# meijieru/AtomNAS

Hardware: AMD Instinct MI355X
Metric: images/sec (whole node) AtomNAS-C supernet 224x224 bs256/GPU (higher is better)
Workload: dtype bf16; 1 GPU; atomnas_c_supernet full training step (fwd + CE-smooth/L2/L1 + bwd + grad all-reduce + RMSprop + EMA), 224x224; per_gpu_batch=256, global_batch=256, parallelism=dp1, hip_graph=True

## Files before the change

### atomnas_amd/csrc/pwconv_tn.hip

```cpp
#include "pwconv.h"

namespace atomnas {

constexpr int UT_MAX = 20;
constexpr int TN_ROWS = 32;

template <typename T, int UMODE, int VMODE>
__global__ __launch_bounds__(256) void k_gemm_tn(Operand U, int NU, Operand V, int NV, float* __restrict__ out, long si, long sj,
                                                 long M, long rows_per_block, float* __restrict__ ws) {
  using MM = Mma<T>;
  constexpr int E = MM::EPL;
  constexpr int SUB = TN_ROWS / (4 * E);
  constexpr int UP = 16 * UT_MAX + 2;
  constexpr int VP = 64 + 2;
  __shared__ T s_u[TN_ROWS * UP];
  __shared__ T s_v[TN_ROWS * VP];

  const int tid = threadIdx.x;
  const int lane = tid & 63, wave = tid >> 6;
  const int q = lane >> 4, j = lane & 15;

  const int u0 = blockIdx.z * (16 * UT_MAX);
  const int nu = min(NU - u0, 16 * UT_MAX);
  const int ut = (nu + 15) / 16;
  const int v0 = blockIdx.y * 64;
  const int nv = min(NV - v0, 64);
  const long r_beg = (long)blockIdx.x * rows_per_block;
  const long r_end = min(M, r_beg + rows_per_block);

  f32x4 acc[UT_MAX];
#pragma unroll
  for (int t = 0; t < UT_MAX; ++t) acc[t] = f32x4{0.f, 0.f, 0.f, 0.f};

  const int ugroups = (ut * 16) / E;
  const int vgroups = 64 / E;

  for (long r0 = r_beg; r0 < r_end; r0 += TN_ROWS) {
    for (int idx = tid; idx < TN_ROWS * ugroups; idx += 256) {
      const int rr = idx / ugroups, cg = (idx % ugroups) * E;
      float v[E];
      load_pro<T, UMODE>(U, r0 + rr, (r0 + rr) < r_end, u0 + cg, NU, v);
#pragma unroll
      for (int e = 0; e < E; ++e) s_u[rr * UP + cg + e] = from_f32<T>(v[e]);
    }
    for (int idx = tid; idx < TN_ROWS * vgroups; idx += 256) {
      const int rr = idx / vgroups, cg = (idx % vgroups) * E;
      float v[E];
      load_pro<T, VMODE>(V, r0 + rr, (r0 + rr) < r_end, v0 + cg, NV, v);
#pragma unroll
      for (int e = 0; e < E; ++e) s_v[rr * VP + cg + e] = from_f32<T>(v[e]);
    }
    __syncthreads();

#pragma unroll
    for (int sb = 0; sb < SUB; ++sb) {
      float bv[E];
#pragma unroll
      for (int e = 0; e < E; ++e) bv[e] = to_f32(s_v[(4 * E * sb + E * q + e) * VP + 16 * wave + j]);
      const typename MM::frag bf = MM::pack(bv);
#pragma unroll
      for (int t = 0; t < UT_MAX; ++t) {
        if (t < ut) {
          float uv[E];
#pragma unroll
          for (int e = 0; e < E; ++e) uv[e] = to_f32(s_u[(4 * E * sb + E * q + e) * UP + 16 * t + j]);
          acc[t] = MM::mma(MM::pack(uv), bf, acc[t]);
        }
      }
    }
    __syncthreads();
  }

  const int vc = v0 + 16 * wave + j;
  if (vc < NV) {
#pragma unroll
    for (int t = 0; t < UT_MAX; ++t) {
      if (t < ut) {
#pragma unroll
        for (int r = 0; r < 4; ++r) {
          const int uc = u0 + 16 * t + 4 * q + r;
          if (uc < NU) {
            if (ws) ws[((long)blockIdx.x * NU + uc) * NV + vc] = acc[t][r];
            else out[uc * si + vc * sj] += acc[t][r];
          }
        }
      }
    }
  }
}


template <int UMODE, int VMODE, int UTT, int VTT, int ROWS>
__global__ __launch_bounds__(256) void k_gemm_tn2(Operand U, int NU, Operand V, int NV, float* __restrict__ out, long si, long sj, long M,
                                                  long rows_per_block, int nchunks, int vt, int uz, int xcd_aware, float* __restrict__ ws) {
  using T = bf16_t;
  using MM = Mma<T>;
  constexpr int VW = 64 * VTT;
  constexpr int RP = ROWS + 8;
  extern __shared__ __attribute__((aligned(16))) unsigned char smem_raw[];
  T* s_v = reinterpret_cast<T*>(smem_raw);
  T* s_u = s_v + VW * RP;
  float* s_cv = reinterpret_cast<float*>(s_u + 16 * UTT * RP);
  float* s_cu = s_cv + 3 * VW;

  const int tid = threadIdx.x;
  const int lane = tid & 63, wave = tid >> 6;
  const int q = lane >> 4, j = lane & 15;
  const int ntile = vt * uz;
  int tile; long chunk;
  if (xcd_aware) {
    const int b_xcd = blockIdx.x & 7, b_local = blockIdx.x >> 3;
    tile = b_local % ntile;
    chunk = (long)(b_local / ntile) * 8 + b_xcd;
  } else {
    chunk = blockIdx.x % nchunks;
    tile = blockIdx.x / nchunks;
    if (tile >= ntile) return;
  }
  if (chunk >= nchunks) return;
  const int u0 = (tile / vt) * (16 * UTT);
  const int nu = min(NU - u0, 16 * UTT);
  const int ut = (nu + 15) / 16;
  const int v0 = (tile % vt) * VW;
  const long r_beg = chunk * rows_per_block;
  const long r_end = min(M, r_beg + rows_per_block);

  f32x4 acc[VTT][UTT];
#pragma unroll
  for (int v = 0; v < VTT; ++v)
#pragma unroll
    for (int t = 0; t < UTT; ++t) acc[v][t] = f32x4{0.f, 0.f, 0.f, 0.f};

  stage_coeffs<VMODE>(V, v0, VW, NV, s_cv, tid);
  stage_coeffs<UMODE>(U, u0, 16 * UTT, NU, s_cu, tid);
  __syncthreads();

  const int ugroups = ut * 2;
  constexpr int NVU = ((ROWS / 2) * (VW / 8) + 255) / 256;
  constexpr int NUU = ((ROWS / 2) * (2 * UTT) + 255) / 256;
  constexpr bool V2 = VMODE == PRO_BNBWD, U2 = UMODE == PRO_BNBWD;
  bf16x8 rva[NVU][2], rvx[V2 ? NVU : 1][2], rua[NUU][2], rux[U2 ? NUU : 1][2];
  const int K8V = (NV + 7) & ~7, K8U = (NU + 7) & ~7;
  auto unit = [&](int idx, bool slab, int& cg, int& rp) {
    if (slab) {
      const int u = idx >> 1;
      rp = u % (ROWS / 2);
      cg = (u / (ROWS / 2)) * 2 + (idx & 1);
    } else {
      rp = idx % (ROWS / 2); cg = idx / (ROWS / 2);
    }
  };
  const bool vslab = V.ss1 != 0, uslab = U.ss1 != 0;
  const long v_m1 = V.ss1 ? 16 : V.ld1, v_m2 = V.ss2 ? 16 : V.ld2, u_m1 = U.ss1 ? 16 : U.ld1, u_m2 = U.ss2 ? 16 : U.ld2;
  auto v_unit = [&](int i, int& rp, long& c1, long& c2) {
    int cg;
    const int idx = tid + 256 * i;
    unit(idx < (ROWS / 2) * (VW / 8) ? idx : 0, vslab, cg, rp);
    int k = v0 + cg * 8;
    k = k < NV ? k : K8V - 8;
    c1 = lay_off(0, k, V.ld1, V.ss1);
    c2 = V2 ? lay_off(0, k, V.ld2, V.ss2) : 0;
  };
  auto u_unit = [&](int i, int& rp, long& c1, long& c2) {
    int cg;
    const int idx = tid + 256 * i;
    unit(idx < (ROWS / 2) * ugroups ? idx : 0, uslab, cg, rp);
    int k = u0 + cg * 8;
    k = k < NU ? k : K8U - 8;
    c1 = lay_off(0, k, U.ld1, U.ss1);
    c2 = U2 ? lay_off(0, k, U.ld2, U.ss2) : 0;
  };
  constexpr bool RUNP = !(U2 && UTT >= 20);
  const T* pv1[NVU]; const T* pv2[V2 ? NVU : 1]; const T* pu1[NUU]; const T* pu2[U2 ? NUU : 1];
#pragma unroll
  for (int i = 0; i < NVU; ++i) {
    int rp; long c1, c2;
    v_unit(i, rp, c1, c2);
    pv1[i] = reinterpret_cast<const T*>(V.p1) + ((r_beg + 2 * rp) * v_m1 + c1);
    if constexpr (V2) pv2[i] = reinterpret_cast<const T*>(V.p2) + ((r_beg + 2 * rp) * v_m2 + c2);
  }
#pragma unroll
  for (int i = 0; i < NUU; ++i) {
    int rp; long c1, c2;
    u_unit(i, rp, c1, c2);
    pu1[i] = reinterpret_cast<const T*>(U.p1) + ((r_beg + 2 * rp) * u_m1 + c1);
    if constexpr (U2) pu2[i] = reinterpret_cast<const T*>(U.p2) + ((r_beg + 2 * rp) * u_m2 + c2);
  }
  long r_run = r_beg;
  auto issue = [&](long r0) {
    if (RUNP && r0 == r_run && r0 + ROWS <= M) {
#pragma unroll
      for (int i = 0; i < NVU; ++i) {
        rva[i][0] = *reinterpret_cast<const bf16x8*>(pv1[i]);
        rva[i][1] = *reinterpret_cast<const bf16x8*>(pv1[i] + v_m1);
        pv1[i] += ROWS * v_m1;
        if constexpr (V2) {
          rvx[i][0] = *reinterpret_cast<const bf16x8*>(pv2[i]);
          rvx[i][1] = *reinterpret_cast<const bf16x8*>(pv2[i] + v_m2);
          pv2[i] += ROWS * v_m2;
        }
      }
#pragma unroll
      for (int i = 0; i < NUU; ++i) {
        rua[i][0] = *reinterpret_cast<const bf16x8*>(pu1[i]);
        rua[i][1] = *reinterpret_cast<const bf16x8*>(pu1[i] + u_m1);
        pu1[i] += ROWS * u_m1;
        if constexpr (U2) {
          rux[i][0] = *reinterpret_cast<const bf16x8*>(pu2[i]);
          rux[i][1] = *reinterpret_cast<const bf16x8*>(pu2[i] + u_m2);
          pu2[i] += ROWS * u_m2;
        }
      }
      r_run = r0 + ROWS;
      return;
    }
#pragma unroll
    for (int i = 0; i < NVU; ++i) {
      int rp; long c1, c2;
      v_unit(i, rp, c1, c2);
#pragma unroll
      for (int h = 0; h < 2; ++h) {
        long r = r0 + 2 * rp + h;
        r = r < M ? r : M - 1;
        rva[i][h] = *reinterpret_cast<const bf16x8*>(reinterpret_cast<const T*>(V.p1) + (r * v_m1 + c1));
        if constexpr (V2) rvx[i][h] = *reinterpret_cast<const bf16x8*>(reinterpret_cast<const T*>(V.p2) + (r * v_m2 + c2));
      }
    }
#pragma unroll
    for (int i = 0; i < NUU; ++i) {
      int rp; long c1, c2;
      u_unit(i, rp, c1, c2);
#pragma unroll
      for (int h = 0; h < 2; ++h) {
        long r = r0 + 2 * rp + h;
        r = r < M ? r : M - 1;
        rua[i][h] = *reinterpret_cast<const bf16x8*>(reinterpret_cast<const T*>(U.p1) + (r * u_m1 + c1));
        if constexpr (U2) rux[i][h] = *reinterpret_cast<const bf16x8*>(reinterpret_cast<const T*>(U.p2) + (r * u_m2 + c2));
      }
    }
  };
  auto xform = [&](auto mode_tag, const Operand& o, const bf16x8& ra, const bf16x8& rx, bool guard, bool valid, const float* lc1,
                   const float* lc2, const float* lc3, float (&v)[8]) {
    constexpr int MODE = decltype(mode_tag)::value;
#pragma unroll
    for (int e = 0; e < 8; ++e) v[e] = (float)ra[e];
    if constexpr (MODE == PRO_BNRELU) {
      float sc[8], sh[8];
      VecIO<float, 8>::load(lc1, sc);
      VecIO<float, 8>::load(lc2, sh);
#pragma unroll
      for (int e = 0; e < 8; ++e) v[e] = v[e] * sc[e] + sh[e];
      act_apply_v<8>(v, act_of(o.relu));
    } else if constexpr (MODE == PRO_BNBWD) {
      float a1[8], a2[8], a3[8];
      VecIO<float, 8>::load(lc1, a1);
      VecIO<float, 8>::load(lc2, a2);
      VecIO<float, 8>::load(lc3, a3);
#pragma unroll
      for (int e = 0; e < 8; ++e) v[e] = a1[e] * v[e] + a2[e] * (float)rx[e] + a3[e];
    }
    if (guard) {
#pragma unroll
      for (int e = 0; e < 8; ++e) v[e] = valid ? v[e] : 0.f;
    }
  };
  const bool v_tail = VMODE == PRO_NONE && v0 + VW > NV, u_tail = UMODE == PRO_NONE && u0 + 16 * UTT > NU;
  auto stage = [&](long r0) {
    const bool row_guard = r0 + ROWS > r_end;
#pragma unroll
    for (int i = 0; i < NVU; ++i) {
      int cg, rp;
      const int idx = tid + 256 * i;
      const bool active = idx < (ROWS / 2) * (VW / 8);
      unit(active ? idx : 0, vslab, cg, rp);
      float a[8], bb[8];
      const float* lc = s_cv + cg * 8;
      const bool kv = v0 + cg * 8 < NV;
      xform(std::integral_constant<int, VMODE>{}, V, rva[i][0], rvx[V2 ? i : 0][0], row_guard || v_tail, kv && (r0 + 2 * rp) < r_end, lc, lc + VW, lc + 2 * VW, a);
      xform(std::integral_constant<int, VMODE>{}, V, rva[i][1], rvx[V2 ? i : 0][1], row_guard || v_tail, kv && (r0 + 2 * rp + 1) < r_end, lc, lc + VW, lc + 2 * VW, bb);
      if (active) {
        T* d = s_v + (((2 * rp) >> 5) * (VW / 16) + (cg >> 1)) * 512 + ((2 * rp) & 31) * 16 + (cg & 1) * 8;
        *reinterpret_cast<bf16x8*>(d) = MM::pack(a);
        *reinterpret_cast<bf16x8*>(d + 16) = MM::pack(bb);
      }
    }
#pragma unroll
    for (int i = 0; i < NUU; ++i) {
      int cg, rp;
      const int idx = tid + 256 * i;
      const bool active = idx < (ROWS / 2) * ugroups;
      unit(active ? idx : 0, uslab, cg, rp);
      float a[8], bb[8];
      const float* lc = s_cu + cg * 8;
      const bool kv = u0 + cg * 8 < NU;
      xform(std::integral_constant<int, UMODE>{}, U, rua[i][0], rux[U2 ? i : 0][0], row_guard || u_tail, kv && (r0 + 2 * rp) < r_end, lc, lc + 16 * UTT, lc + 32 * UTT, a);
      xform(std::integral_constant<int, UMODE>{}, U, rua[i][1], rux[U2 ? i : 0][1], row_guard || u_tail, kv && (r0 + 2 * rp + 1) < r_end, lc, lc + 16 * UTT, lc + 32 * UTT, bb);
      if (active) {
        T* d = s_u + (((2 * rp) >> 5) * UTT + (cg >> 1)) * 512 + ((2 * rp) & 31) * 16 + (cg & 1) * 8;
        *reinterpret_cast<bf16x8*>(d) = MM::pack(a);
        *reinterpret_cast<bf16x8*>(d + 16) = MM::pack(bb);
      }
    }
  };
  const unsigned tr_lane = (unsigned)(((8 * q + (j >> 2)) * 16 + 4 * (j & 3)) * 2);
  auto tr_frag = [&](const T* sub) {
    const unsigned a0 = (unsigned)(size_t)((__attribute__((address_space(3))) const char*)sub) + tr_lane;
    bf16x4 lo, hi;
    asm volatile("ds_read_b64_tr_b16 %0, %1" : "=v"(lo) : "v"(a0) : "memory");
    asm volatile("ds_read_b64_tr_b16 %0, %1 offset:128" : "=v"(hi) : "v"(a0) : "memory");
    return TrFrag{lo, hi};
  };
  issue(r_beg);
  for (long r0 = r_beg; r0 < r_end; r0 += ROWS) {
    stage(r0);
    issue(r0 + ROWS);
    __syncthreads();
#pragma unroll 2
    for (int ks = 0; ks < ROWS / 32; ++ks) {
      TrFrag bfp[VTT], afp[UTT];
#pragma unroll
      for (int v = 0; v < VTT; ++v) bfp[v] = tr_frag(s_v + (ks * (VW / 16) + 4 * v + wave) * 512);
#pragma unroll
      for (int t = 0; t < UTT; ++t)
        if (t < ut) afp[t] = tr_frag(s_u + (ks * UTT + t) * 512);
      asm volatile("s_waitcnt lgkmcnt(0)" ::: "memory");
      __builtin_amdgcn_sched_barrier(0);
      bf16x8 bf[VTT];
#pragma unroll
      for (int v = 0; v < VTT; ++v) bf[v] = __builtin_shufflevector(bfp[v].lo, bfp[v].hi, 0, 1, 2, 3, 4, 5, 6, 7);
#pragma unroll
      for (int t = 0; t < UTT; ++t) {
        if (t < ut) {
          const bf16x8 af = __builtin_shufflevector(afp[t].lo, afp[t].hi, 0, 1, 2, 3, 4, 5, 6, 7);
#pragma unroll
          for (int v = 0; v < VTT; ++v) acc[v][t] = MM::mma(af, bf[v], acc[v][t]);
        }
      }
    }
    __syncthreads();
  }

#pragma unroll
  for (int v = 0; v < VTT; ++v) {
    const int vc = v0 + 64 * v + 16 * wave + j;
    if (vc < NV) {
#pragma unroll
      for (int t = 0; t < UTT; ++t) {
        if (t < ut) {
#pragma unroll
          for (int r = 0; r < 4; ++r) {
            const int uc = u0 + 16 * t + 4 * q + r;
            if (uc < NU) {
              if (ws) ws[(chunk * NU + uc) * NV + vc] = acc[v][t][r];
              else out[uc * si + vc * sj] += acc[v][t][r];
            }
          }
        }
      }
    }
  }
}

template <int UTT, bool VPRO, int TN3_DEPTH>
__global__ __launch_bounds__(256, 2) void k_gemm_tn3(Operand U, int NU, Operand V, int NV, float* __restrict__ out, long si, long sj, long M,
                                                  long rows_per_block, int nchunks, int vt, int uz, float* __restrict__ ws) {
  using T = bf16_t;
  using MM = Mma<T>;
  constexpr int NSUB = 8 + UTT;
  constexpr int DPS = (NSUB + 3) / 4;
  constexpr int STAGE = NSUB * 512;
  extern __shared__ __attribute__((aligned(16))) unsigned char smem_raw[];
  T* s_st = reinterpret_cast<T*>(smem_raw);

  const int tid = threadIdx.x;
  const int lane = tid & 63, wave = __builtin_amdgcn_readfirstlane(tid >> 6);
  const int q = lane >> 4, j = lane & 15;
  const int ntile = vt * uz;
  const int b_xcd = blockIdx.x & 7, b_local = blockIdx.x >> 3;
  const int tile = b_local % ntile;
  const long chunk = (long)(b_local / ntile) * 8 + b_xcd;
  if (chunk >= nchunks) return;
  const int u0 = (tile / vt) * (16 * UTT);
  const int nu = min(NU - u0, 16 * UTT);
  const int ut = (nu + 15) / 16;
  const int v0 = (tile % vt) * 128;
  const long r_beg = chunk * rows_per_block;
  const long r_end = min(M, r_beg + rows_per_block);
  const int nstages = (int)((r_end - r_beg + 31) / 32);

  const int r_l = lane >> 1, h_l = lane & 1;
  long src_off[DPS], src_mul[DPS];
  const T* src_base[DPS];
  unsigned dst_off[DPS];
#pragma unroll
  for (int i = 0; i < DPS; ++i) {
    int sub = wave + 4 * i;
    sub = sub < NSUB ? sub : NSUB - 1;
    dst_off[i] = (unsigned)sub * 1024u;
    if (sub < 8) {
      int c = v0 + 16 * sub + 8 * h_l;
      c = c < ((NV + 7) & ~7) ? c : 0;
      src_base[i] = reinterpret_cast<const T*>(V.p1);
      src_off[i] = lay_off(0, c, V.ld1, V.ss1);
      src_mul[i] = V.ss1 ? 16 : V.ld1;
    } else {
      int c = u0 + 16 * (sub - 8) + 8 * h_l;
      c = c < ((NU + 7) & ~7) ? c : 0;
      src_base[i] = reinterpret_cast<const T*>(U.p1);
      src_off[i] = lay_off(0, c, U.ld1, U.ss1);
      src_mul[i] = U.ss1 ? 16 : U.ld1;
    }
  }
  const unsigned lds0 = (unsigned)(size_t)((__attribute__((address_space(3))) const char*)s_st);
  auto copy_stage = [&](int s) {
    const int sc = s < nstages ? s : nstages - 1;
    long row = r_beg + 32L * sc + r_l;
    row = row < M ? row : M - 1;
    const unsigned slot = lds0 + (unsigned)(s % TN3_DEPTH) * (unsigned)(STAGE * 2);
#pragma unroll
    for (int i = 0; i < DPS; ++i) {
      const T* g = src_base[i] + (row * src_mul[i] + src_off[i]);
      const unsigned d = __builtin_amdgcn_readfirstlane(slot + dst_off[i]);
      unsigned keep;
      asm volatile("s_mov_b32 %0, m0\n\ts_mov_b32 m0, %2\n\ts_nop 0\n\tglobal_load_lds_dwordx4 %1, off\n\ts_mov_b32 m0, %0"
                   : "=&s"(keep) : "v"(g), "s"(d) : "memory");
    }
    ATOMNAS_RING_STAGE_END();
  };

  float vsc[2] = {1.f, 1.f}, vsh[2] = {0.f, 0.f};
  if constexpr (VPRO) {
#pragma unroll
    for (int v = 0; v < 2; ++v) {
      const int c = v0 + 64 * v + 16 * wave + j;
      if (c < NV) { vsc[v] = V.c1[c]; vsh[v] = V.c2[c]; }
    }
  }
  const Act vact = act_of(V.relu);

  f32x4 acc[2][UTT];
#pragma unroll
  for (int v = 0; v < 2; ++v)
#pragma unroll
    for (int t = 0; t < UTT; ++t) acc[v][t] = f32x4{0.f, 0.f, 0.f, 0.f};

  const unsigned tr_lane = (unsigned)(((8 * q + (j >> 2)) * 16 + 4 * (j & 3)) * 2);
  auto tr_frag = [&](unsigned sub_addr) {
    const unsigned a0 = sub_addr + tr_lane;
    bf16x4 lo, hi;
    asm volatile("ds_read_b64_tr_b16 %0, %1" : "=v"(lo) : "v"(a0) : "memory");
    asm volatile("ds_read_b64_tr_b16 %0, %1 offset:128" : "=v"(hi) : "v"(a0) : "memory");
    return TrFrag{lo, hi};
  };

#pragma unroll
  for (int s = 0; s < TN3_DEPTH - 1; ++s) copy_stage(s);
  for (int s = 0; s < nstages; ++s) {
    asm volatile("s_waitcnt vmcnt(%0)" ::"n"((TN3_DEPTH - 2) * DPS) : "memory");
    __syncthreads();
    copy_stage(s + TN3_DEPTH - 1);
    const unsigned slot = lds0 + (unsigned)(s % TN3_DEPTH) * (unsigned)(STAGE * 2);
    TrFrag bfp[2], afp[UTT];
#pragma unroll
    for (int v = 0; v < 2; ++v) bfp[v] = tr_frag(slot + (unsigned)(4 * v + wave) * 1024u);
#pragma unroll
    for (int t = 0; t < UTT; ++t)
      if (t < ut) afp[t] = tr_frag(slot + (unsigned)(8 + t) * 1024u);
    asm volatile("s_waitcnt lgkmcnt(0)" ::: "memory");
    __builtin_amdgcn_sched_barrier(0);
    bf16x8 bf[2];
#pragma unroll
    for (int v = 0; v < 2; ++v) {
      bf[v] = __builtin_shufflevector(bfp[v].lo, bfp[v].hi, 0, 1, 2, 3, 4, 5, 6, 7);
      if constexpr (VPRO) {
        float x[8];
#pragma unroll
        for (int e = 0; e < 8; ++e) x[e] = (float)bf[v][e] * vsc[v] + vsh[v];
        act_apply_v<8>(x, vact);
        bf[v] = MM::pack(x);
      }
    }
    const long rows_left = r_end - (r_beg + 32L * s);
#pragma unroll
    for (int t = 0; t < UTT; ++t) {
      if (t < ut) {
        bf16x8 af = __builtin_shufflevector(afp[t].lo, afp[t].hi, 0, 1, 2, 3, 4, 5, 6, 7);
        if (rows_left < 32) {
#pragma unroll
          for (int e = 0; e < 8; ++e)
            if (8 * q + e >= rows_left) af[e] = (bf16_t)0.f;
        }
#pragma unroll
        for (int v = 0; v < 2; ++v) acc[v][t] = MM::mma(af, bf[v], acc[v][t]);
      }
    }
  }
  asm volatile("s_waitcnt vmcnt(0)" ::: "memory");

#pragma unroll
  for (int v = 0; v < 2; ++v) {
    const int vc = v0 + 64 * v + 16 * wave + j;
    if (vc < NV) {
#pragma unroll
      for (int t = 0; t < UTT; ++t) {
        if (t < ut) {
#pragma unroll
          for (int r = 0; r < 4; ++r) {
            const int uc = u0 + 16 * t + 4 * q + r;
            if (uc < NU) {
              if (ws) ws[(chunk * NU + uc) * NV + vc] = acc[v][t][r];
              else out[uc * si + vc * sj] += acc[v][t][r];
            }
          }
        }
      }
    }
  }
}

struct TnArgs {
  int umode; Operand U; int NU;
  int vmode; Operand V; int NV;
  float* out; long si, sj, M;
  float* ws; long ws_floats;
  hipStream_t st;
};

template <int... Vs, typename F> static int for_value(int v, F&& f) {
  int rc = 1;
  (void)((v == Vs ? (rc = f(IC<Vs>{}), true) : false) || ...);
  return rc;
}
template <typename F> static int for_pair(int umode, int vmode, F&& f) {
#define X(UM, VM) if (umode == UM && vmode == VM) return f(IC<UM>{}, IC<VM>{});
  X(PRO_NONE, PRO_NONE) X(PRO_NONE, PRO_BNBWD) X(PRO_BNBWD, PRO_BNRELU) X(PRO_BNRELU, PRO_BNBWD) X(PRO_BNBWD, PRO_NONE)
  X(PRO_NONE, PRO_BNRELU)
#undef X
  set_error("gemm_tn: unsupported prologue pair (%d,%d)", umode, vmode);
  return 1;
}

static int tn_utt(int NU, bool dma) {
  const int ut = (NU + 15) / 16;
  return ut <= 2 ? (dma ? 4 : 2) : ut <= 4 ? 4 : ut <= 6 ? 6 : ut <= 12 ? 12 : ut <= 20 ? 10 : 20;
}

static long tn_ws_cap(const TnArgs& a) { return a.ws ? a.ws_floats / ((long)a.NU * a.NV) : 1; }
static void tn_split(long M, long want, long min_rows, long quantum, long& chunks, long& rows) {
  if (want < 1) want = 1;
  rows = (M + want - 1) / want;
  if (rows < min_rows) rows = min_rows;
  rows = (rows + quantum - 1) / quantum * quantum;
  chunks = (M + rows - 1) / rows;
}
static int tn_finish(const char* what, const TnArgs& a, long chunks) {
  if (int rc = check_launch(what)) return rc;
  if (chunks > 1) return reduce_parts(a.ws, (long)a.NU * a.NV, (int)chunks, (long)a.NU * a.NV, a.out, a.NV, a.si, a.sj, a.st);
  return 0;
}

using TnDmaKernel = decltype(&k_gemm_tn3<4, false, 4>);
struct TnDmaPlan { TnDmaKernel kern; int utt, vt, uz; size_t lds; long chunks, rows; unsigned grid; };
constexpr int DMA_MINNU = 32, DMA_MINNV = 256;
constexpr long DMA_MINM = 1024, DMA_MINROWS = 128;
constexpr int tn3_depth(int utt) { return 2 * (4 * (8 + utt) * 1024) + 4096 <= 160 * 1024 ? 4 : 3; }
static bool tn_dma_plan(const TnArgs& a, TnDmaPlan& p) {
  static const int on = getenv("ATOMNAS_TN_DMA") ? atoi(getenv("ATOMNAS_TN_DMA")) : 1;
  if (!on || a.umode != PRO_NONE || (a.vmode != PRO_NONE && a.vmode != PRO_BNRELU) || !a.ws) return false;
  if (a.NV < DMA_MINNV || a.NU < DMA_MINNU || a.M < DMA_MINM) return false;
  p.utt = tn_utt(a.NU, true);
  if (for_value<4, 6, 12, 10>(p.utt, [&](auto utt) {
        constexpr int UTT = decltype(utt)::value, DEPTH = tn3_depth(UTT);
        p.kern = a.vmode == PRO_BNRELU ? k_gemm_tn3<UTT, true, DEPTH> : k_gemm_tn3<UTT, false, DEPTH>;
        p.lds = (size_t)DEPTH * (8 + UTT) * 1024;
        return 0;
      }))
    return false;
  if (p.lds > max_lds_bytes()) return false;
  p.vt = (a.NV + 127) / 128, p.uz = (a.NU + 16 * p.utt - 1) / (16 * p.utt);
  const long tiles = (long)p.vt * p.uz;
  long want = (long)num_cus() * resident_per_cu(p.kern, 256, p.lds) / tiles;
  if (want > a.M / DMA_MINROWS) want = a.M / DMA_MINROWS;
  if (want > tn_ws_cap(a)) want = tn_ws_cap(a);
  want = want / 8 * 8;
  if (want < 8) return false;
  tn_split(a.M, want, 0, 32, p.chunks, p.rows);
  p.grid = (unsigned)((p.chunks + 7) / 8 * 8 * tiles);
  return true;
}
static int tn_dma_launch(const TnDmaPlan& p, const TnArgs& a) {
  hipLaunchKernelGGL(p.kern, dim3(p.grid), dim3(256), p.lds, a.st, a.U, a.NU, a.V, a.NV, a.out, a.si, a.sj, a.M, p.rows, (int)p.chunks, p.vt,
                     p.uz, a.ws);
  return tn_finish("gemm_tn3", a, p.chunks);
}

using TnSlabKernel = decltype(&k_gemm_tn2<PRO_NONE, PRO_NONE, 2, 1, 128>);
struct TnSlabPlan { TnSlabKernel kern; int utt, vtt, slab_rows, vt, uz; size_t lds; long chunks, rows; int xcd; unsigned grid; };
constexpr int SLAB_WIDE_MINNV = 256;
static bool tn_slab_plan(const TnArgs& a, TnSlabPlan& p) {
  p.utt = tn_utt(a.NU, false);
  const bool wide = p.utt >= 4 && p.utt <= 12 && a.NV >= SLAB_WIDE_MINNV;
  p.vtt = wide ? 2 : 1, p.slab_rows = wide ? 64 : 128;
  if (for_pair(a.umode, a.vmode, [&](auto um, auto vm) {
        return for_value<2, 4, 6, 12, 10, 20>(p.utt, [&](auto utt) {
          constexpr int UM = decltype(um)::value, VM = decltype(vm)::value, UTT = decltype(utt)::value;
          p.kern = k_gemm_tn2<UM, VM, UTT, 1, 128>;
          if constexpr (UTT >= 4 && UTT <= 12)
            if (wide) p.kern = k_gemm_tn2<UM, VM, UTT, 2, 64>;
          return 0;
        });
      }))
    return false;
  const int vw = 64 * p.vtt, uw = 16 * p.utt;
  p.vt = (a.NV + vw - 1) / vw, p.uz = (a.NU + uw - 1) / uw;
  p.lds = (size_t)(vw + uw) * (p.slab_rows + 8) * sizeof(bf16_t) + (size_t)3 * (vw + uw) * sizeof(float);
  const long tiles = (long)p.vt * p.uz;
  long want = (long)num_cus() * resident_per_cu(p.kern, 256, p.lds) / tiles;
  if (want > a.M / (2 * p.slab_rows)) want = a.M / (2 * p.slab_rows);
  if (want > tn_ws_cap(a)) want = tn_ws_cap(a);
  p.xcd = want >= 8;
  if (p.xcd) want = want / 8 * 8;
  tn_split(a.M, want, 0, 1, p.chunks, p.rows);
  p.grid = (unsigned)((p.xcd ? (p.chunks + 7) / 8 * 8 : p.chunks) * tiles);
  return true;
}
static int tn_slab_launch(const TnSlabPlan& p, const TnArgs& a) {
  hipLaunchKernelGGL(p.kern, dim3(p.grid), dim3(256), p.lds, a.st, a.U, a.NU, a.V, a.NV, a.out, a.si, a.sj, a.M, p.rows, (int)p.chunks, p.vt,
                     p.uz, p.xcd, p.chunks > 1 ? a.ws : nullptr);
  return tn_finish("gemm_tn2", a, p.chunks);
}

using TnGenericKernel = decltype(&k_gemm_tn<float, PRO_NONE, PRO_NONE>);
struct TnGenericPlan { TnGenericKernel kern; int vt, uz; long chunks, rows; };
static bool tn_generic_plan(const TnArgs& a, TnGenericPlan& p) {
  if (for_pair(a.umode, a.vmode, [&](auto um, auto vm) { p.kern = k_gemm_tn<float, decltype(um)::value, decltype(vm)::value>; return 0; }))
    return false;
  p.vt = (a.NV + 63) / 64, p.uz = (a.NU + 16 * UT_MAX - 1) / (16 * UT_MAX);
  const long tiles = (long)p.vt * p.uz;
  long want = (1024 + tiles - 1) / tiles;
  if (want > tn_ws_cap(a)) want = tn_ws_cap(a);
  tn_split(a.M, want, 8 * TN_ROWS, TN_ROWS, p.chunks, p.rows);
  return true;
}
static int tn_generic_launch(const TnGenericPlan& p, const TnArgs& a) {
  hipLaunchKernelGGL(p.kern, dim3((unsigned)p.chunks, p.vt, p.uz), dim3(256), 0, a.st, a.U, a.NU, a.V, a.NV, a.out, a.si, a.sj, a.M, p.rows,
                     p.chunks > 1 ? a.ws : nullptr);
  return tn_finish("gemm_tn", a, p.chunks);
}

static int launch_tn(const TnArgs& a, int dtype) {
  TnDmaPlan dma; TnSlabPlan slab; TnGenericPlan generic;
  if (dtype == DT_BF16 && tn_dma_plan(a, dma)) return tn_dma_launch(dma, a);
  if (dtype == DT_BF16 && tn_slab_plan(a, slab)) return tn_slab_launch(slab, a);
  if (dtype == DT_F32 && tn_generic_plan(a, generic)) return tn_generic_launch(generic, a);
  return 1;
}

}

using namespace atomnas;

extern "C" int atomnas_pw_gemm_tn(int u_mode, const void* u, int ldu, long u_ss, const void* u2, int ldu2, long u2_ss, const float* uc1,
                                  const float* uc2, const float* uc3, int u_relu, int NU, int v_mode, const void* v, int ldv, long v_ss,
                                  const void* v2, int ldv2, long v2_ss, const float* vc1, const float* vc2, const float* vc3, int v_relu, int NV, float* out,
                                  long si, long sj, long M, float* ws, long ws_floats, int dtype, void* stream) {
  ATOMNAS_REQUIRE(dtype == DT_F32 || dtype == DT_BF16, "pw_gemm_tn: bad dtype %d", dtype);
  ATOMNAS_REQUIRE(M > 0 && NU > 0 && NV > 0 && out, "pw_gemm_tn: empty shape");
  Operand U{u, ldu, u2, ldu2, u_ss, u2_ss, uc1, uc2, uc3, u_relu};
  Operand V{v, ldv, v2, ldv2, v_ss, v2_ss, vc1, vc2, vc3, v_relu};
  ATOMNAS_REQUIRE((u_ss == 0 || u_ss >= M * 16) && (v_ss == 0 || v_ss >= M * 16), "pw_gemm_tn: slab stride smaller than M*16");
  if (check_operand("pw_gemm_tn(U)", U, u_mode, NU)) return 1;
  if (check_operand("pw_gemm_tn(V)", V, v_mode, NV)) return 1;
  return launch_tn(TnArgs{u_mode, U, NU, v_mode, V, NV, out, si, sj, M, ws, ws_floats, (hipStream_t)stream}, dtype);
}
```

Measured before the change: 9628 images/sec.

## Add k-split variant of slab TN weight-gradient GEMM for tiny channel counts

```diff
diff --git a/atomnas_amd/csrc/pwconv_tn.hip b/atomnas_amd/csrc/pwconv_tn.hip
--- a/atomnas_amd/csrc/pwconv_tn.hip
+++ b/atomnas_amd/csrc/pwconv_tn.hip
@@ -90,12 +90,13 @@
 }
 
 
-template <int UMODE, int VMODE, int UTT, int VTT, int ROWS>
+template <int UMODE, int VMODE, int UTT, int VTT, int ROWS, bool KSPLIT = false>
 __global__ __launch_bounds__(256) void k_gemm_tn2(Operand U, int NU, Operand V, int NV, float* __restrict__ out, long si, long sj, long M,
                                                   long rows_per_block, int nchunks, int vt, int uz, int xcd_aware, float* __restrict__ ws) {
   using T = bf16_t;
   using MM = Mma<T>;
-  constexpr int VW = 64 * VTT;
+  static_assert(!KSPLIT || (ROWS == 128 && VTT == 2 && UTT == 2), "k_gemm_tn2<KSPLIT>: four k-steps for four waves, 2 x 2 tiles per wave");
+  constexpr int VW = KSPLIT ? 32 : 64 * VTT;
   constexpr int RP = ROWS + 8;
   extern __shared__ __attribute__((aligned(16))) unsigned char smem_raw[];
   T* s_v = reinterpret_cast<T*>(smem_raw);
@@ -316,10 +317,10 @@
     issue(r0 + ROWS);
     __syncthreads();
 #pragma unroll 2
-    for (int ks = 0; ks < ROWS / 32; ++ks) {
+    for (int ks = KSPLIT ? wave : 0; ks < (KSPLIT ? wave + 1 : ROWS / 32); ++ks) {
       TrFrag bfp[VTT], afp[UTT];
 #pragma unroll
-      for (int v = 0; v < VTT; ++v) bfp[v] = tr_frag(s_v + (ks * (VW / 16) + 4 * v + wave) * 512);
+      for (int v = 0; v < VTT; ++v) bfp[v] = tr_frag(s_v + (ks * (VW / 16) + (KSPLIT ? v : 4 * v + wave)) * 512);
 #pragma unroll
       for (int t = 0; t < UTT; ++t)
         if (t < ut) afp[t] = tr_frag(s_u + (ks * UTT + t) * 512);
@@ -340,9 +341,30 @@
     __syncthreads();
   }
 
+  if constexpr (KSPLIT) {
+    f32x4* s_acc = reinterpret_cast<f32x4*>(smem_raw);
+    if (wave > 0) {
+#pragma unroll
+      for (int v = 0; v < VTT; ++v)
+#pragma unroll
+        for (int t = 0; t < UTT; ++t) s_acc[((wave - 1) * (VTT * UTT) + v * UTT + t) * 64 + lane] = acc[v][t];
+    }
+    __syncthreads();
+    if (wave > 0) return;
+#pragma unroll
+    for (int w = 1; w < 4; ++w)
+#pragma unroll
+      for (int v = 0; v < VTT; ++v)
+#pragma unroll
+        for (int t = 0; t < UTT; ++t) {
+          const f32x4 o = s_acc[((w - 1) * (VTT * UTT) + v * UTT + t) * 64 + lane];
+#pragma unroll
+          for (int r = 0; r < 4; ++r) acc[v][t][r] += o[r];
+        }
+  }
 #pragma unroll
   for (int v = 0; v < VTT; ++v) {
-    const int vc = v0 + 64 * v + 16 * wave + j;
+    const int vc = KSPLIT ? v0 + 16 * v + j : v0 + 64 * v + 16 * wave + j;
     if (vc < NV) {
 #pragma unroll
       for (int t = 0; t < UTT; ++t) {
@@ -595,23 +617,28 @@
 }
 
 using TnSlabKernel = decltype(&k_gemm_tn2<PRO_NONE, PRO_NONE, 2, 1, 128>);
-struct TnSlabPlan { TnSlabKernel kern; int utt, vtt, slab_rows, vt, uz; size_t lds; long chunks, rows; int xcd; unsigned grid; };
+struct TnSlabPlan { TnSlabKernel kern; int utt, vtt, slab_rows, vw, vt, uz; size_t lds; long chunks, rows; int xcd; unsigned grid; };
 constexpr int SLAB_WIDE_MINNV = 256;
+constexpr int SLAB_KSPLIT_MAXN = 32;
+constexpr long SLAB_KSPLIT_MINM = 65536;
 static bool tn_slab_plan(const TnArgs& a, TnSlabPlan& p) {
   p.utt = tn_utt(a.NU, false);
   const bool wide = p.utt >= 4 && p.utt <= 12 && a.NV >= SLAB_WIDE_MINNV;
-  p.vtt = wide ? 2 : 1, p.slab_rows = wide ? 64 : 128;
+  const bool ksplit = a.NV <= SLAB_KSPLIT_MAXN && a.NU <= SLAB_KSPLIT_MAXN && a.M >= SLAB_KSPLIT_MINM;
+  p.vtt = wide || ksplit ? 2 : 1, p.slab_rows = wide ? 64 : 128, p.vw = ksplit ? 32 : 64 * p.vtt;
   if (for_pair(a.umode, a.vmode, [&](auto um, auto vm) {
         return for_value<2, 4, 6, 12, 10, 20>(p.utt, [&](auto utt) {
           constexpr int UM = decltype(um)::value, VM = decltype(vm)::value, UTT = decltype(utt)::value;
           p.kern = k_gemm_tn2<UM, VM, UTT, 1, 128>;
           if constexpr (UTT >= 4 && UTT <= 12)
             if (wide) p.kern = k_gemm_tn2<UM, VM, UTT, 2, 64>;
+          if constexpr (UTT == 2)
+            if (ksplit) p.kern = k_gemm_tn2<UM, VM, 2, 2, 128, true>;
           return 0;
         });
       }))
     return false;
-  const int vw = 64 * p.vtt, uw = 16 * p.utt;
+  const int vw = p.vw, uw = 16 * p.utt;
   p.vt = (a.NV + vw - 1) / vw, p.uz = (a.NU + uw - 1) / uw;
   p.lds = (size_t)(vw + uw) * (p.slab_rows + 8) * sizeof(bf16_t) + (size_t)3 * (vw + uw) * sizeof(float);
   const long tiles = (long)p.vt * p.uz;
```

New measurement: 9659 images/sec (median of 6 runs). No clear change (+0.3%).
